# anshumang/gunrockINST

Hardware: AMD Instinct MI355X
Metric: MTEPS (million traversed edges/sec) BFS R-MAT scale-24 (higher is better)
Workload: dtype int32; 1 GPU; BFS idempotent direction-optimizing (traversal_mode 2), R-MAT scale-24 (a=.55 b=.2 c=.2 d=.05, 8 pairs/vertex mirrored, seed 0x6772): n=16777216, m=265395436 directed edges; sources: largest-degree + 64 seeded; search_depth_src0=7, max_degree=218420

## Files before the change

### gunrockinst_amd/csrc/gunrock/app/bfs/bfs_enactor.hpp

```cpp
#pragma once

#include <hip/hip_runtime.h>
#include <cstdlib>

#include <gunrock/app/bfs/bfs_functor.hpp>
#include <gunrock/app/bfs/bfs_problem.hpp>
#include <gunrock/app/enactor_base.hpp>
#include <gunrock/oprtr/advance/bottom_up.hpp>
#include <gunrock/oprtr/advance/kernel.hpp>
#include <gunrock/oprtr/advance/twc.hpp>
#include <gunrock/util/context.hpp>

namespace gunrock {
namespace app {
namespace bfs {

template <bool INSTRUMENT>
class BFSEnactor : public EnactorBase {
   public:
    explicit BFSEnactor(bool DEBUG = false) : EnactorBase(VERTEX_FRONTIERS, DEBUG) {}
    ~BFSEnactor() override {}

    void GetKernelStatistics(long long &launches, double &kernel_ms)
    {
// ... 188 lines not shown
                    if (scap > cu_count * 4) scap = cu_count * 4;
                    if (sgrid > scap) sgrid = scap;
                    hipLaunchKernelGGL((oprtr::advance::BottomUpSparseKernel<BU_THREADS, 8, 32, BFSProblem, L, true>),
                                       dim3(static_cast<unsigned>(sgrid)), dim3(BU_THREADS), 0, stream, bargs, *ds, lookup);
                    queue_emitted = true;
                    return util::GRError("BottomUpSparseKernel launch failed", __FILE__, __LINE__);
                }
                const long long scap = max_grid_size > 0 ? max_grid_size
                    : util::ResidentGrid(oprtr::advance::BottomUpSparseKernel<BU_THREADS, 8, 32, BFSProblem, L, false>, BU_THREADS);
                if (sgrid > scap) sgrid = scap;
                hipLaunchKernelGGL((oprtr::advance::BottomUpSparseKernel<BU_THREADS, 8, 32, BFSProblem, L, false>),
                                   dim3(static_cast<unsigned>(sgrid)), dim3(BU_THREADS), 0, stream, bargs, *ds, lookup);
                return util::GRError("BottomUpSparseKernel launch failed", __FILE__, __LINE__);
            }
            if (heads_only) {
                typedef oprtr::advance::BitmapLookup<VertexId> L;
                const long long hcap = max_grid_size > 0 ? max_grid_size : util::ResidentGrid(oprtr::advance::BottomUpHeadsKernel<BU_THREADS, BFSProblem, L>, BU_THREADS);
                if (grid > hcap) grid = hcap;
                if (grid < 1) grid = 1;
                hipLaunchKernelGGL((oprtr::advance::BottomUpHeadsKernel<BU_THREADS, BFSProblem, L>), dim3(static_cast<unsigned>(grid)), dim3(BU_THREADS), 0,
                                   stream, bargs, *ds, lookup);
                return util::GRError("BottomUpHeadsKernel launch failed", __FILE__, __LINE__);
            }
            const long long cap = max_grid_size > 0 ? max_grid_size
                : util::ResidentGrid(oprtr::advance::BottomUpKernel<BU_THREADS, 8, 32, BFSProblem, oprtr::advance::BitmapLookup<VertexId>>, BU_THREADS);
            if (grid > cap) grid = cap;
            if (grid < 1) grid = 1;
            hipLaunchKernelGGL((oprtr::advance::BottomUpKernel<BU_THREADS, 8, 32, BFSProblem, oprtr::advance::BitmapLookup<VertexId>>),
                               dim3(static_cast<unsigned>(grid)), dim3(BU_THREADS), 0, stream, bargs, *ds, lookup);
            return util::GRError("BottomUpKernel launch failed", __FILE__, __LINE__);
        };
        const int chain_len = (dobfs && problem->chain_sweeps > 0)
            ? (problem->chain_sweeps < oprtr::advance::kChainMax ? problem->chain_sweeps : oprtr::advance::kChainMax) : 0;
        work_progress.publish_sets = chain_len > 0 ? chain_len + 1 : 1;
        oprtr::advance::SweepRule sweep_rule;
        sweep_rule.with_in_edges = problem->with_in_edges;
        sweep_rule.nodes = problem->nodes;
        sweep_rule.beta = problem->beta;
        sweep_rule.emit_factor = problem->emit_queue_factor;
        sweep_rule.sparse_div = problem->sparse_sweep_div;
        auto run_sweep_chain = [&](long long first_in) -> hipError_t {
            typedef oprtr::advance::BitmapLookup<VertexId> L;
            hipError_t rc = hipSuccess;
            const long long it0 = iteration;
            const long long base_total = enactor_stats.total_queued;
            int masks[oprtr::advance::kChainMax + 1];
            masks[0] = cur_mask;
            int queued = 0;
            const long long bu_steps = ((static_cast<long long>(problem->nodes) + 63) / 64 + oprtr::advance::kBottomUpStepWords - 1) / oprtr::advance::kBottomUpStepWords;
            long long grid = (bu_steps + (BU_THREADS / 64) - 1) / (BU_THREADS / 64);
            const long long cap = max_grid_size > 0 ? max_grid_size
                : util::ResidentGrid(oprtr::advance::BottomUpAutoKernel<BU_THREADS, 8, 32, BFSProblem, L>, BU_THREADS);
            if (grid > cap) grid = cap;
            if (grid < 1) grid = 1;
            const long long chunks = ((static_cast<long long>(problem->nodes) + 63) / 64 + oprtr::advance::kSparseChunkWords - 1) / oprtr::advance::kSparseChunkWords;
            long long sparse_grid = (chunks + (BU_THREADS / 64) - 1) / (BU_THREADS / 64);
            if (sparse_grid < 1) sparse_grid = 1;
            long long emit_grid = sparse_grid < cu_count * 4 ? sparse_grid : cu_count * 4;
            for (int k = 1; k <= chain_len; ++k) {
                bool got = false;
                if ((rc = problem->TryAcquireMask(stream, masks[k], masks, k, got))) return rc;
                if (!got) break;
                oprtr::advance::BottomUpArgs<VertexId, SizeT> bargs;
                bargs.nodes = problem->nodes;
                bargs.d_inv_row_offsets = ds->d_inv_row_offsets;
                bargs.d_inv_column_indices = ds->d_inv_column_indices;
                bargs.d_inv_heads = ds->d_inv_heads;
                L lookup{ds->d_frontier_mask[masks[k - 1]]};
                bargs.d_frontier_out = reinterpret_cast<unsigned long long *>(ds->d_frontier_mask[masks[k]]);
                bargs.d_visited = reinterpret_cast<unsigned long long *>(ds->d_visited_mask);
                const long long level = it0 + k - 1;
                bargs.d_tail_out = work_progress.d_tail + ((level + 1) & 3);
                bargs.d_tail_clear = work_progress.d_tail + ((level + 2) & 3);
                bargs.d_wide = work_progress.d_wide + static_cast<size_t>(k) * util::WorkProgress::kWideSetWords;
                bargs.head_skip = 0;
                bargs.heads_only = 0;
                bargs.d_never = reinterpret_cast<const unsigned long long *>(ds->d_never_mask);
                bargs.d_head_base = ds->d_head_base;
                bargs.d_duty = INSTRUMENT ? DutySlot() : nullptr;
                bargs.queue_out = gs->frontier_queues[selector];
                bargs.d_fwd_row_offsets = gs->d_row_offsets;
                bargs.d_queue_tail = work_progress.d_tail + ((level + 1) & 3);
                bargs.d_queue_invalid = reinterpret_cast<int *>(work_progress.AuxTail());
                bargs.d_overflow = work_progress.d_overflow;
                oprtr::advance::SweepChain chain;
                chain.d_sets = work_progress.d_wide;
                chain.base_total = base_total;
                chain.first_in = first_in;
                chain.rule = sweep_rule;
                chain.index = k;
                chain.first_may_switch = 0;
                chain.d_log = work_progress.d_chain_log;
                typename BFSProblem::DataSlice level_slice = *ds;
                level_slice.iteration = static_cast<VertexId>(level);
                hipLaunchKernelGGL((oprtr::advance::BottomUpAutoKernel<BU_THREADS, 8, 32, BFSProblem, L>), dim3(static_cast<unsigned>(grid)),
                                   dim3(BU_THREADS), 0, stream, bargs, level_slice, lookup, chain, static_cast<unsigned>(sparse_grid),
                                   static_cast<unsigned>(emit_grid));
                if ((rc = util::GRError("BottomUpAutoKernel launch failed", __FILE__, __LINE__))) return rc;
                queued = k;
            }
            if (queued == 0) return util::GRError(hipErrorInvalidValue, "BFSEnactor: no frontier bitmap for a bottom-up sweep", __FILE__, __LINE__);
            const bool closing_queued = problem->chain_closing && problem->persistent_edge_limit > 0;
            int *d_gate = work_progress.d_chain_log + 8;
            bool emit_queued = false;
            if (closing_queued) {
                oprtr::advance::PersistentArgs<VertexId, SizeT> p;
                p.t.queue[0] = gs->frontier_queues[0];
                p.t.queue[1] = gs->frontier_queues[1];
                p.t.selector = selector;
                p.t.first_iteration = it0;
                p.t.d_tail = work_progress.d_tail;
                p.t.max_levels = kTailMaxLevels;
                p.t.d_levels_done = work_progress.LevelsDone();
                p.t.d_level_sums = work_progress.d_sums;
                p.t.d_row_offsets = gs->d_row_offsets;
                p.t.d_column_indices = gs->d_column_indices;
                p.t.d_overflow = work_progress.d_overflow;
                p.t.edge_limit = static_cast<SizeT>(static_cast<long long>(problem->persistent_edge_limit) * 4);
                p.barrier.d_counter = work_progress.BarrierCounter();
                p.barrier.d_timeout = work_progress.BarrierTimeout();
// ... 368 lines not shown
```

### gunrockinst_amd/csrc/gunrock/app/bfs/bfs_problem.hpp

```cpp
#pragma once

#include <hip/hip_runtime.h>

#include <gunrock/app/problem_base.hpp>
#include <gunrock/graphio/device_csr.hpp>
#include <gunrock/graphio/relabel.hpp>
#include <gunrock/oprtr/advance/binned.hpp>
#include <gunrock/oprtr/advance/bottom_up.hpp>
#include <gunrock/util/memset_kernel.hpp>

namespace gunrock {
namespace app {
namespace bfs {

template <typename SizeT>
__global__ void NoInEdgeMaskKernel(const SizeT *d_inv_row_offsets, long long nodes, long long words64, unsigned long long *d_mask)
{
    const unsigned lane = threadIdx.x & 63;
    const long long wave0 = (static_cast<long long>(blockIdx.x) * blockDim.x + threadIdx.x) / 64;
    const long long nwaves = static_cast<long long>(gridDim.x) * blockDim.x / 64;
    for (long long w = wave0; w < words64; w += nwaves) {
        const long long v = w * 64 + lane;
        const bool none = v < nodes && d_inv_row_offsets[v + 1] == d_inv_row_offsets[v];
        const unsigned long long m = __ballot(none);
// ... 809 lines not shown
        }
        return src_row[1] - src_row[0];
    }

    hipError_t Extract(VertexId *h_labels, VertexId *h_preds)
    {
        hipError_t retval = hipSuccess;
        hipStream_t stream = this->graph_slices[0]->stream;
        GR_CHECK(FinishSearch(stream), "BFSProblem Extract: label pass failed");
        GR_CHECK(hipStreamSynchronize(stream), "BFSProblem Extract sync failed");
        if (this->nodes > 0)
            GR_CHECK(hipMemcpy(h_labels, d_out_labels, sizeof(VertexId) * static_cast<size_t>(this->nodes), hipMemcpyDeviceToHost),
                     "BFSProblem hipMemcpy d_labels failed");
        if (MARK_PREDECESSORS && h_preds && this->nodes > 0)
            GR_CHECK(hipMemcpy(h_preds, d_out_preds, sizeof(VertexId) * static_cast<size_t>(this->nodes), hipMemcpyDeviceToHost),
                     "BFSProblem hipMemcpy d_preds failed");
        return retval;
    }

    bool defer_labels = true;
    bool emit_current = false;
    bool labels_deferred = false;
    int label_pass = 1;
    int level_mask_limit = kLevelMasks;
    LevelMaskList<VertexId> level_masks;
    int mask_ring = 0;

    bool MaskKept(int idx) const
    {
        for (int k = 0; k < level_masks.count; ++k)
            if (level_masks.mask[k] == reinterpret_cast<const unsigned long long *>(data_slices[0]->d_frontier_mask[idx])) return true;
        return false;
    }
    hipError_t AcquireMask(hipStream_t stream, int &idx, int hold_a = -1, int hold_b = -1)
    {
        const int holds[2] = {hold_a, hold_b};
        bool got = false;
        const hipError_t rc = TryAcquireMask(stream, idx, holds, 2, got);
        if (rc) return rc;
        return got ? hipSuccess : util::GRError(hipErrorInvalidValue, "BFSProblem: no free frontier bitmap", __FILE__, __LINE__);
    }
    hipError_t TryAcquireMask(hipStream_t stream, int &idx, const int *holds, int n_holds, bool &got)
    {
        hipError_t retval = hipSuccess;
        got = true;
        if (!data_slices[0]->d_frontier_mask[1]) {
// ... 155 lines not shown
```

### gunrockinst_amd/csrc/gunrock/oprtr/advance/bottom_up.hpp

```cpp
#pragma once

#include <hip/hip_runtime.h>

#include <gunrock/oprtr/advance/sweep_chain.hpp>
#include <gunrock/oprtr/frontier_writer.hpp>
#include <gunrock/util/device_intrinsics.hpp>
#include <gunrock/util/error_utils.hpp>
#include <gunrock/util/frontier.hpp>
#include <gunrock/util/kernel_runtime_stats.hpp>

namespace gunrock {
namespace oprtr {
namespace advance {

template <typename VertexId, typename SizeT>
__global__ void QueueToBitmapKernel(const VertexId *d_queue, SizeT length, unsigned *d_bitmap)
{
    const SizeT stride = static_cast<SizeT>(gridDim.x) * blockDim.x;
    for (SizeT i = static_cast<SizeT>(blockIdx.x) * blockDim.x + threadIdx.x; i < length; i += stride) {
        const VertexId v = d_queue[i];
        atomicOr(d_bitmap + (static_cast<unsigned>(v) >> 5), 1u << (v & 31));
    }
}

// ... 115 lines not shown
    unsigned long long *d_queue_tail = nullptr;
    int *d_queue_invalid = nullptr;
    int *d_overflow = nullptr;
    int heads_only = 0;
    unsigned long long *d_wide = nullptr;
    unsigned long long *d_duty = nullptr;
};

#ifndef GRX_BU_STEP_WORDS
#define GRX_BU_STEP_WORDS 8
#endif
constexpr int kBottomUpStepWords = GRX_BU_STEP_WORDS;
#ifndef GRX_BU_SPARSE_CHUNK_WORDS
#define GRX_BU_SPARSE_CHUNK_WORDS 64
#endif
constexpr int kSparseChunkWords = GRX_BU_SPARSE_CHUNK_WORDS;

struct __attribute__((packed, aligned(4))) Quad {
    int v[4];
};

constexpr int kHeadScan = 512;

template <typename VertexId, typename SizeT>
__global__ void BuildHeadsKernel(const SizeT *d_row_offsets, const VertexId *d_column_indices, long long nodes, int2 *d_heads,
                                 const SizeT *d_degree_offsets,
                                 const unsigned long long *d_never = nullptr, const unsigned *d_head_base = nullptr)
{
    const unsigned lane = util::LaneId();
    const long long nwaves = static_cast<long long>(gridDim.x) * blockDim.x / util::kWaveSize;
    for (long long v = (static_cast<long long>(blockIdx.x) * blockDim.x + threadIdx.x) / util::kWaveSize; v < nodes; v += nwaves) {
        const SizeT b = d_row_offsets[v], e = d_row_offsets[v + 1];
        const SizeT len = (e - b < kHeadScan) ? e - b : kHeadScan;
        unsigned long long k1 = 0, k2 = 0;
        for (SizeT i = lane; i < len; i += util::kWaveSize) {
            const VertexId u = d_column_indices[b + i];
            const unsigned long long deg = d_degree_offsets ? static_cast<unsigned long long>(d_degree_offsets[u + 1] - d_degree_offsets[u])
                                                            : static_cast<unsigned long long>(kHeadScan - i);
            const unsigned long long k = ((deg + 1) << 32) | static_cast<unsigned>(u);
            if (k > k1) { k2 = k1; k1 = k; }
            else if (k > k2) k2 = k;
        }
        unsigned long long best1 = k1;
        for (int o = 32; o; o >>= 1) {
            const unsigned long long other = __shfl_xor(best1, o, util::kWaveSize);
            best1 = other > best1 ? other : best1;
        }
        unsigned long long best2 = (k1 == best1) ? k2 : k1;
        for (int o = 32; o; o >>= 1) {
            const unsigned long long other = __shfl_xor(best2, o, util::kWaveSize);
            best2 = other > best2 ? other : best2;
        }
        if (lane == 0) {
            int2 h;
            h.x = best1 ? static_cast<int>(static_cast<unsigned>(best1)) : -1;
            h.y = best2 ? static_cast<int>(static_cast<unsigned>(best2)) : -1;
            if (!d_head_base) {
                d_heads[v] = h;
            } else if (e > b) {
                const unsigned long long with_edges = ~d_never[v >> 6];
                d_heads[d_head_base[v >> 6] + __popcll(with_edges & ((1ull << (v & 63)) - 1ull))] = h;
            }
        }
    }
}

template <int PROBE, int SOLO_LIMIT, typename VertexId, typename SizeT, typename Lookup>
__device__ __forceinline__ VertexId WalkRow(const BottomUpArgs<VertexId, SizeT> &a, const Lookup &in_frontier, bool active, VertexId v,
                                            unsigned lane, VertexId known_a = -1, VertexId known_b = -1, bool extent_given = false,
                                            SizeT given_begin = 0, SizeT given_end = 0)
{
    SizeT pos = 0, end = 0;
    VertexId p_found = -1;
    if (extent_given) {
        pos = given_begin + a.head_skip;
        end = given_end;
    } else if (active) {
        pos = a.d_inv_row_offsets[v] + a.head_skip;
        end = a.d_inv_row_offsets[v + 1];
// ... 113 lines not shown
                    head[j] = a.d_inv_heads[open ? idx : 0u];
                }
            } else {
#pragma unroll
                for (int j = 0; j < STEP_WORDS; ++j) {
                    const unsigned long long open_mask = __shfl(my_open, j, util::kWaveSize);
                    const bool open = (open_mask >> lane) & 1ull;
                    open_bits |= static_cast<unsigned>(open) << j;
                    const long long v = (step * STEP_WORDS + j) * 64 + lane;
                    head[j] = a.d_inv_heads[open ? v : 0];
                }
            }
            bool hit[STEP_WORDS];
#pragma unroll
            for (int j = 0; j < STEP_WORDS; ++j) {
                const bool ask = ((open_bits >> j) & 1u) && head[j].x >= 0;
                hit[j] = in_frontier(ask ? head[j].x : 0) && ask;
            }
            VertexId parent[STEP_WORDS];
            unsigned ask_y = 0;
#pragma unroll
            for (int j = 0; j < STEP_WORDS; ++j) {
                parent[j] = hit[j] ? head[j].x : static_cast<VertexId>(-1);
                if (((open_bits >> j) & 1u) && head[j].x >= 0 && !hit[j] && head[j].y >= 0) ask_y |= 1u << j;
            }
            unsigned more_bits = 0;
            if (__ballot(ask_y != 0) != 0) {
#pragma unroll
                for (int j = 0; j < STEP_WORDS; ++j) {
                    const bool ask = (ask_y >> j) & 1u;
                    hit[j] = in_frontier(ask ? head[j].y : 0) && ask;
                }
#pragma unroll
                for (int j = 0; j < STEP_WORDS; ++j) {
                    if (hit[j]) parent[j] = head[j].y;
                    if (((ask_y >> j) & 1u) && !hit[j]) more_bits |= 1u << j;
                }
            }

            if (HEADS_ONLY || a.heads_only) more_bits = 0;
            typedef typename ProblemData::SizeT SizeT;
            SizeT next_begin = 0, next_end = 0;
            if (!HEADS_ONLY && more_bits != 0) {
                const long long nv = (step * STEP_WORDS + (__ffs(more_bits) - 1)) * 64 + lane;
                next_begin = a.d_inv_row_offsets[nv];
                next_end = a.d_inv_row_offsets[nv + 1];
            }
            while (!HEADS_ONLY && __ballot(more_bits != 0) != 0) {
                const bool active = more_bits != 0;
                const int jl = active ? (__ffs(more_bits) - 1) : 0;
                more_bits &= more_bits - 1;
                const VertexId v = static_cast<VertexId>((step * STEP_WORDS + jl) * 64 + lane);
                const SizeT row_begin = next_begin, row_end = next_end;
                if (more_bits != 0) {
                    const long long nv = (step * STEP_WORDS + (__ffs(more_bits) - 1)) * 64 + lane;
                    next_begin = a.d_inv_row_offsets[nv];
                    next_end = a.d_inv_row_offsets[nv + 1];
                }
                VertexId hx = -1, hy = -1;
// ... 30 lines not shown
                const unsigned long long fm = __ballot(found);
                if (static_cast<int>(lane) == j) my_found |= fm;
            }
        }
        if (owns_word) {
            a.d_frontier_out[my_word] = my_found;
            if (my_found) a.d_visited[my_word] = my_vis | my_found;
        }
    }

    unsigned long long packed = util::PackTail(found_count, found_edges);
    packed = util::WaveSum(packed);
    if (lane == 0) s_total[tid / util::kWaveSize] = packed;
    __syncthreads();
    if (tid == 0) {
        unsigned long long sum = 0;
#pragma unroll
        for (int i = 0; i < WAVES; ++i) sum += s_total[i];
        unsigned long long *slot = util::WideTailSlot(a.d_wide);
        if (sum) atomicAdd(slot ? slot : a.d_tail_out, sum);
    }
}

#ifndef GRX_BU_MIN_WAVES
#define GRX_BU_MIN_WAVES 6
#endif
template <int THREADS, int PROBE, int SOLO_LIMIT, typename ProblemData, typename Lookup>
__global__ __launch_bounds__(THREADS, GRX_BU_MIN_WAVES) void BottomUpKernel(
    BottomUpArgs<typename ProblemData::VertexId, typename ProblemData::SizeT> a, typename ProblemData::DataSlice slice,
    Lookup in_frontier)
{
    DenseSweep<THREADS, PROBE, SOLO_LIMIT, ProblemData, Lookup>(a, slice, in_frontier);
}

#ifndef GRX_BU_HEADS_MIN_WAVES
#define GRX_BU_HEADS_MIN_WAVES 6
#endif
template <int THREADS, typename ProblemData, typename Lookup>
__global__ __launch_bounds__(THREADS, GRX_BU_HEADS_MIN_WAVES) void BottomUpHeadsKernel(
    BottomUpArgs<typename ProblemData::VertexId, typename ProblemData::SizeT> a, typename ProblemData::DataSlice slice,
    Lookup in_frontier)
{
    DenseSweep<THREADS, 8, 32, ProblemData, Lookup, true>(a, slice, in_frontier);
}

__device__ __forceinline__ int NthSetBit(unsigned long long x, int r)
{
    int pos = 0;
#pragma unroll
    for (int s = 32; s; s >>= 1) {
        const int c = __popcll(x & (((1ull << s) - 1ull) << pos));
        if (r >= c) {
            r -= c;
            pos += s;
        }
// ... 57 lines not shown
            my_with_edges = ~a.d_never[my_word];
            my_base = a.d_head_base[my_word];
        }
        for (int i = lane; i < CHUNK_WORDS * 2; i += util::kWaveSize) s_found[wave][i] = 0;
        __builtin_amdgcn_wave_barrier();

        for (unsigned base = 0; base < total; base += util::kWaveSize) {
            const unsigned k = base + lane;
            const bool active = k < total;
            int j = 0;
#pragma unroll
            for (int s = CHUNK_WORDS / 2; s; s >>= 1)
                if (__shfl(inc, j + s - 1, util::kWaveSize) <= k) j += s;
            if (!active) j = 0;
            const unsigned before = __shfl(inc, j, util::kWaveSize) - __shfl(cnt, j, util::kWaveSize);
            const unsigned long long open_j = __shfl(my_open, j, util::kWaveSize);
            const int bit = active ? NthSetBit(open_j, static_cast<int>(k - before)) : 0;
            const VertexId v = static_cast<VertexId>((chunk * CHUNK_WORDS + j) * 64 + bit);
            long long head_index = v;
            if (a.d_head_base) {
                const unsigned long long we = __shfl(my_with_edges, j, util::kWaveSize);
                head_index = __shfl(my_base, j, util::kWaveSize) + __popcll(we & ((1ull << bit) - 1ull));
            }
            const int2 head = a.d_inv_heads[active ? head_index : 0];
            VertexId parent = -1;
            const bool ask_x = active && head.x >= 0;
            const bool hit_x = in_frontier(ask_x ? head.x : 0) && ask_x;
            if (hit_x) parent = head.x;
            const bool ask_y = ask_x && !hit_x && head.y >= 0;
            bool more = false;
            if (__ballot(ask_y) != 0) {
                const bool hit_y = in_frontier(ask_y ? head.y : 0) && ask_y;
                if (hit_y) parent = head.y;
                more = ask_y && !hit_y;
            }
            if (a.heads_only) more = false;
            if (__ballot(more) != 0) {
                const VertexId late = WalkRow<PROBE, SOLO_LIMIT>(a, in_frontier, more, v, lane, head.x, head.y);
                if (more && late >= 0) parent = late;
            }
            if (parent >= 0) {
                if (!slice.defer_labels) slice.d_labels[v] = new_label;
                if (ProblemData::MARK_PREDECESSORS) slice.d_preds[v] = parent;
                atomicOr(&s_found[wave][2 * j + (bit >> 5)], 1u << (bit & 31));
            }
            if (EMIT_QUEUE && emit) {
                const unsigned long long fm = __ballot(parent >= 0);
                if (fm) {
                    const int leader = __ffsll(static_cast<long long>(fm)) - 1;
                    int at = 0;
                    if (static_cast<int>(lane) == leader) at = atomicAdd(&s_writer.count, __popcll(fm));
                    at = __shfl(at, leader, util::kWaveSize);
                    if (parent >= 0 && at + __popcll(fm) <= CAPACITY) s_writer.buf[at + util::RankInMask(fm)] = v;
                }
            }
        }
        __builtin_amdgcn_wave_barrier();
// ... 16 lines not shown
        for (int i = 0; i < WAVES; ++i) sum += s_total[i];
        unsigned long long *slot = util::WideTailSlot(a.d_wide);
        if (sum) atomicAdd(slot ? slot : a.d_tail_out, sum);
    }
    if (EMIT_QUEUE && emit) {
        const int staged = Writer::Count(s_writer);
        __syncthreads();
        if (staged > CAPACITY) {
            if (tid == 0) *a.d_queue_invalid = 1;
        } else {
            Writer::template Flush<true>(s_writer, staged, a.queue_out, a.d_queue_tail, a.d_overflow, a.d_fwd_row_offsets);
        }
    }
}

template <int THREADS, int PROBE, int SOLO_LIMIT, typename ProblemData, typename Lookup, bool EMIT_QUEUE>
__global__ __launch_bounds__(THREADS) void BottomUpSparseKernel(
    BottomUpArgs<typename ProblemData::VertexId, typename ProblemData::SizeT> a, typename ProblemData::DataSlice slice,
    Lookup in_frontier)
{
    SparseSweep<THREADS, PROBE, SOLO_LIMIT, ProblemData, Lookup, EMIT_QUEUE>(a, slice, in_frontier, EMIT_QUEUE, gridDim.x);
}

template <int THREADS, int PROBE, int SOLO_LIMIT, typename ProblemData, typename Lookup>
__global__ __launch_bounds__(THREADS, GRX_BU_MIN_WAVES) void BottomUpAutoKernel(
    BottomUpArgs<typename ProblemData::VertexId, typename ProblemData::SizeT> a, typename ProblemData::DataSlice slice,
    Lookup in_frontier, SweepChain chain, unsigned sparse_grid, unsigned emit_grid)
{
    const int action = ChainAction(chain, util::LaneId());
    if (blockIdx.x == 0 && threadIdx.x == 0) {
        chain.d_log[chain.index] = action;
        if (action >= kSweepDense && action != kSweepSparseEmit && a.d_queue_tail) *a.d_queue_tail = 0ull;
    }
    if (action < kSweepDense) return;
    if (action == kSweepDense) {
        DenseSweep<THREADS, PROBE, SOLO_LIMIT, ProblemData, Lookup>(a, slice, in_frontier);
    } else {
        const unsigned want = action == kSweepSparseEmit ? emit_grid : sparse_grid;
        const unsigned limit = want < gridDim.x ? want : gridDim.x;
        if (blockIdx.x >= limit) return;
        SparseSweep<THREADS, PROBE, SOLO_LIMIT, ProblemData, Lookup, true>(a, slice, in_frontier, action == kSweepSparseEmit, limit);
    }
}

template <int THREADS, typename VertexId, typename SizeT>
__global__ __launch_bounds__(THREADS) void BitmapToQueueKernel(const unsigned *d_bitmap, SizeT nodes,
                                                               util::Frontier<VertexId, SizeT> out,
                                                               unsigned long long *d_tail_out, int *d_overflow,
                                                               const SizeT *d_row_offsets)
{
    constexpr int CAPACITY = 16 * THREADS;
    constexpr int WAVES = THREADS / util::kWaveSize;
    typedef FrontierWriter<THREADS, CAPACITY, VertexId, SizeT> Writer;
    __shared__ typename Writer::Storage s_writer;
    __shared__ unsigned s_pop[WAVES];

    const long long words = (static_cast<long long>(nodes) + 31) / 32;
    const long long per_wg = ((words + gridDim.x - 1) / gridDim.x + THREADS - 1) / THREADS * THREADS;
    const long long w_begin = static_cast<long long>(blockIdx.x) * per_wg;
// ... 66 lines not shown
```

### gunrockinst_amd/csrc/lib/bfs_app.hip

```cpp
#include <gunrock/gunrock.h>
#include <gunrock/gunrock_mi355x.h>

#include <cstdio>
#include <cstdlib>

#include <gunrock/app/bfs/bfs_enactor.hpp>
#include <gunrock/app/bfs/bfs_problem.hpp>
#include <gunrock/app/handle_runner.hpp>
#include <gunrock/graphio/device_sort.hpp>
#include <gunrock/graphio/symmetry.hpp>
#include <gunrock/oprtr/filter/kernel.hpp>
#include <gunrock/csr.hpp>
#include <gunrock/graphio/utils.hpp>
#include <gunrock/util/context.hpp>

using namespace gunrock;
using namespace gunrock::app;
using namespace gunrock::app::bfs;

namespace {

struct BfsRunner {
    virtual ~BfsRunner() {}
    virtual hipError_t Init(const Csr<int, int, int> &g) = 0;
// ... 76 lines not shown
    }
    void FreeInverse()
    {
        if (d_inv_row_offsets) util::GRError(hipFree(d_inv_row_offsets), "BFS hipFree inverse offsets failed", __FILE__, __LINE__);
        if (d_inv_column_indices) util::GRError(hipFree(d_inv_column_indices), "BFS hipFree inverse columns failed", __FILE__, __LINE__);
        d_inv_row_offsets = nullptr;
        d_inv_column_indices = nullptr;
    }
    int *d_inv_row_offsets = nullptr;
    int *d_inv_column_indices = nullptr;
    void SetPersistentLimit(int limit) override { problem.persistent_edge_limit = limit; }
    void SetTwcLimit(int limit) override { problem.twc_edge_limit = limit; }
    void SetCooperativeLaunch(bool on) override { problem.cooperative_launch = on; }
    void SetBinnedMinEdges(long long min_edges) override { problem.binned_min_edges = min_edges; }
    int SetOption(const char *name, double value) override
    {
        const std::string key(name ? name : "");
        if (key == "emit_queue_factor") problem.emit_queue_factor = static_cast<float>(value);
        else if (key == "sparse_sweep_div") problem.sparse_sweep_div = static_cast<int>(value);
        else if (key == "speculative_emit") problem.speculative_emit = value != 0.0;
        else if (key == "chain_sweeps") problem.chain_sweeps = static_cast<int>(value);
        else if (key == "chain_closing") problem.chain_closing = value != 0.0;
        else if (key == "label_pass") problem.label_pass = value != 0.0 ? 1 : 0;
        else if (key == "relabel") {
            if (value > 0.0 && !problem.HasRelabelled()) return 2;
            problem.relabel = value > 0.0 ? 1 : (value < 0.0 ? -1 : 0);
        } else if (key == "relabel_min_nodes") {
            if (value < 0.0) return 2;
            problem.relabel_min_nodes = static_cast<long long>(value);
        } else if (key == "relabel_hubs") {
            if (value < 0.0) return 2;
            const long long hubs = static_cast<long long>(value);
            if (!problem.HasRelabelled()) problem.relabel_hubs = hubs;
            else if (hubs != problem.relabel_hubs && problem.BuildRelabelled(hubs) != hipSuccess) return 3;
        } else return 1;
        return 0;
    }
    void BuildRelabelled(bool on) override { problem.build_relabelled = on; }
    long long MaskFlushes() override { return problem.mask_flushes; }
    void RelabelInfo(long long &hubs, long long &with_edges, int &threshold, float &build_ms, long long &bytes) override
    {
        const bool ready = problem.HasRelabelled();
        hubs = ready ? problem.relabelled.hubs : -1;
        with_edges = ready ? problem.relabelled.with_edges : -1;
        threshold = ready ? problem.relabelled.threshold : 0;
        build_ms = ready ? problem.relabelled.build_ms : 0.f;
// ... 358 lines not shown
```

### gunrockinst_amd/csrc/lib/partitioned_bfs.hip

```cpp
#include <gunrock/gunrock_mi355x.h>

#include <dlfcn.h>
#include <cstdio>
#include <cstring>
#include <string>
#include <vector>

#include <gunrock/app/bfs/bfs_problem.hpp>
#include <gunrock/app/enactor_base.hpp>
#include <gunrock/app/problem_base.hpp>
#include <gunrock/graphio/device_sort.hpp>
#include <gunrock/oprtr/advance/bottom_up.hpp>
#include <gunrock/oprtr/advance/kernel.hpp>
#include <gunrock/oprtr/filter/kernel.hpp>
#include <gunrock/util/memset_kernel.hpp>

using namespace gunrock;

namespace {

struct ncclUniqueIdBytes {
    char internal[128];
};

// ... 390 lines not shown
    {
        if (hipStreamSynchronize(stream) != hipSuccess) return -1;
        return gather(ctx, d_send, d_recv, words);
    }
    int AllToAllV(const int *d_send, const size_t *sc, const size_t *so, int *d_recv, const size_t *rc, const size_t *ro,
                  hipStream_t stream) override
    {
        if (hipStreamSynchronize(stream) != hipSuccess) return -1;
        return a2a(ctx, d_send, sc, so, d_recv, rc, ro);
    }
    const char *Name() const override { return "callbacks"; }
};

struct Pbfs : app::EnactorBase {
    int parts = 1, rank = 0;
    int n_global = 0, n_local = 0, n_local_max = 0, m_local = 0;
    int *d_row_offsets = nullptr, *d_col_indices = nullptr;
    PbfsProblem::DataSlice ds{};
    unsigned *d_frontier_mask[2] = {nullptr, nullptr};
    int2 *d_heads = nullptr;
    unsigned *d_never = nullptr;
    unsigned *d_head_base = nullptr;
    long long with_in_edges = 0;
    int sparse_sweep_div = 6;
    bool never_applied = false;
    util::Frontier<int, int> queues[2];
    int *d_candidates = nullptr, *d_send = nullptr;
    unsigned *d_counts = nullptr, *h_counts = nullptr;
    int candidate_capacity = 0;
    hipStream_t stream = 0;
    int selector = 0, cur_mask = 0;
    unsigned frontier_len = 0, frontier_edges = 0;
    int level = 0;
    Transport *transport = nullptr;
    bool mark_pred = false;
    double alpha = 12.0;
    long long m_global = -1;
    int *d_recv = nullptr;
    int recv_capacity = 0;
    int *d_send_preds = nullptr;
    unsigned *d_small = nullptr;
    unsigned *h_small = nullptr;
    unsigned long long mail_seq = 0;
    unsigned *d_mark_bits = nullptr;
    double lite_factor = 230.0;
    long long marked_levels = 0;
// ... 279 lines not shown
        b.head_skip = 0;
        b.d_never = reinterpret_cast<const unsigned long long *>(d_never);
        b.d_head_base = d_head_base;
        b.d_frontier_out = reinterpret_cast<unsigned long long *>(d_frontier_mask[cur_mask ^ 1]);
        b.d_visited = reinterpret_cast<unsigned long long *>(ds.d_visited_mask);
        b.d_tail_out = work_progress.d_tail + 1;
        b.d_tail_clear = nullptr;
        b.d_wide = work_progress.d_wide;
        ds.iteration = level;
        L lookup{d_gathered_masks, static_cast<unsigned>(parts), static_cast<unsigned>(words_per_rank)};
        const long long words64 = (static_cast<long long>(n_local) + 63) / 64;
        if (sparse_sweep_div > 0 && open_estimate >= 0 && open_estimate * sparse_sweep_div <= static_cast<long long>(n_local)) {
            long long sgrid = ((words64 + oprtr::advance::kSparseChunkWords - 1) / oprtr::advance::kSparseChunkWords + 3) / 4;
            const long long scap = util::ResidentGrid(oprtr::advance::BottomUpSparseKernel<256, 8, 32, PbfsProblem, L, false>, 256);
            if (sgrid > scap) sgrid = scap;
            if (sgrid < 1) sgrid = 1;
            hipLaunchKernelGGL((oprtr::advance::BottomUpSparseKernel<256, 8, 32, PbfsProblem, L, false>), dim3(static_cast<unsigned>(sgrid)),
                               dim3(256), 0, stream, b, ds, lookup);
            GR_CHECK(hipGetLastError(), "BottomUpSparseKernel launch failed");
            return retval;
        }
        const long long bu_steps = (words64 + oprtr::advance::kBottomUpStepWords - 1) / oprtr::advance::kBottomUpStepWords;
        long long grid = (bu_steps + 3) / 4;
        const long long cap = util::ResidentGrid(oprtr::advance::BottomUpKernel<256, 8, 32, PbfsProblem, L>, 256);
        if (grid > cap) grid = cap;
        if (grid < 1) grid = 1;
        hipLaunchKernelGGL((oprtr::advance::BottomUpKernel<256, 8, 32, PbfsProblem, L>), dim3(static_cast<unsigned>(grid)), dim3(256), 0, stream,
                           b, ds, lookup);
        GR_CHECK(hipGetLastError(), "BottomUpKernel launch failed");
        return retval;
    }

    hipError_t BitmapToQueue(unsigned *len, unsigned *edges)
    {
        hipError_t retval = hipSuccess;
        if ((retval = work_progress.ClearAux(stream))) return retval;
        hipLaunchKernelGGL((oprtr::advance::BitmapToQueueKernel<256, int, int>), dim3(cu_count * 4), dim3(256), 0, stream,
                           d_frontier_mask[cur_mask], n_local, queues[selector], work_progress.AuxTail(), work_progress.d_overflow,
                           d_row_offsets);
        GR_CHECK(hipGetLastError(), "BitmapToQueueKernel launch failed");
        if ((retval = work_progress.GetAux(frontier_len, frontier_edges, stream))) return retval;
        *len = frontier_len;
        *edges = frontier_edges;
        return retval;
    }

    hipError_t PrepareSearch()
    {
        hipError_t retval = hipSuccess;
        if (!transport) return hipErrorNotInitialized;
        if (!d_small) {
// ... 328 lines not shown
}

int grx_pbfs_labels(grx_pbfs *p, int **d_labels)
{
    if (!p || !d_labels) return -1;
    *d_labels = p->impl.ds.d_labels;
    return 0;
}

int grx_pbfs_preds(grx_pbfs *p, int **d_preds)
{
    if (!p || !d_preds) return -1;
    *d_preds = p->impl.ds.d_preds;
    return 0;
}

int grx_pbfs_set_option(grx_pbfs *p, const char *name, double value)
{
    if (!p || !name) return -1;
    const std::string key(name);
    if (key == "lite_factor") p->impl.lite_factor = value;
    else if (key == "alpha") p->impl.alpha = value;
    else if (key == "sparse_sweep_div") p->impl.sparse_sweep_div = static_cast<int>(value);
    else return 1;
    return 0;
}

long long grx_pbfs_stat(grx_pbfs *p, const char *name)
{
    if (!p || !name) return -1;
    const std::string key(name);
    if (key == "marked_levels") return p->impl.marked_levels;
    return -1;
}

int grx_rccl_load(void)
{
    return RcclApi::Get().Load() ? 0 : -2;
}

int grx_rccl_unique_id(char id[128])
{
    if (!id) return -1;
    RcclApi &api = RcclApi::Get();
    if (!api.Load()) return -2;
    ncclUniqueIdBytes uid;
// ... 52 lines not shown
```

Baseline: 966,300 MTEPS.

## Queue bottom-up row walkers in LDS and drain them wave-wide across batches

Adds a queued dense bottom-up sweep. Vertices whose two cached heads both miss are pushed into a per-wave shared-memory ring and walked together once enough accumulate, instead of walking each step's few unresolved vertices at low lane occupancy. It also encodes in the heads table when the second head is the vertex's last in-edge, so those vertices skip the row walk entirely. The queued path is on by default and adds shared-memory footprint and wave barriers, which may lower occupancy.

```diff
diff --git a/gunrockinst_amd/csrc/gunrock/app/bfs/bfs_enactor.hpp b/gunrockinst_amd/csrc/gunrock/app/bfs/bfs_enactor.hpp
--- a/gunrockinst_amd/csrc/gunrock/app/bfs/bfs_enactor.hpp
+++ b/gunrockinst_amd/csrc/gunrock/app/bfs/bfs_enactor.hpp
@@ -234,12 +234,19 @@
                                    stream, bargs, *ds, lookup);
                 return util::GRError("BottomUpHeadsKernel launch failed", __FILE__, __LINE__);
             }
+            typedef oprtr::advance::BitmapLookup<VertexId> L;
+            const bool walk_queue = problem->walk_queue != 0;
             const long long cap = max_grid_size > 0 ? max_grid_size
-                : util::ResidentGrid(oprtr::advance::BottomUpKernel<BU_THREADS, 8, 32, BFSProblem, oprtr::advance::BitmapLookup<VertexId>>, BU_THREADS);
+                : walk_queue ? util::ResidentGrid(oprtr::advance::BottomUpKernel<BU_THREADS, 8, 32, BFSProblem, L, true>, BU_THREADS)
+                             : util::ResidentGrid(oprtr::advance::BottomUpKernel<BU_THREADS, 8, 32, BFSProblem, L, false>, BU_THREADS);
             if (grid > cap) grid = cap;
             if (grid < 1) grid = 1;
-            hipLaunchKernelGGL((oprtr::advance::BottomUpKernel<BU_THREADS, 8, 32, BFSProblem, oprtr::advance::BitmapLookup<VertexId>>),
-                               dim3(static_cast<unsigned>(grid)), dim3(BU_THREADS), 0, stream, bargs, *ds, lookup);
+            if (walk_queue)
+                hipLaunchKernelGGL((oprtr::advance::BottomUpKernel<BU_THREADS, 8, 32, BFSProblem, L, true>),
+                                   dim3(static_cast<unsigned>(grid)), dim3(BU_THREADS), 0, stream, bargs, *ds, lookup);
+            else
+                hipLaunchKernelGGL((oprtr::advance::BottomUpKernel<BU_THREADS, 8, 32, BFSProblem, L, false>),
+                                   dim3(static_cast<unsigned>(grid)), dim3(BU_THREADS), 0, stream, bargs, *ds, lookup);
             return util::GRError("BottomUpKernel launch failed", __FILE__, __LINE__);
         };
         const int chain_len = (dobfs && problem->chain_sweeps > 0)
@@ -261,8 +268,10 @@
             int queued = 0;
             const long long bu_steps = ((static_cast<long long>(problem->nodes) + 63) / 64 + oprtr::advance::kBottomUpStepWords - 1) / oprtr::advance::kBottomUpStepWords;
             long long grid = (bu_steps + (BU_THREADS / 64) - 1) / (BU_THREADS / 64);
+            const bool walk_queue = problem->walk_queue != 0;
             const long long cap = max_grid_size > 0 ? max_grid_size
-                : util::ResidentGrid(oprtr::advance::BottomUpAutoKernel<BU_THREADS, 8, 32, BFSProblem, L>, BU_THREADS);
+                : walk_queue ? util::ResidentGrid(oprtr::advance::BottomUpAutoKernel<BU_THREADS, 8, 32, BFSProblem, L, true>, BU_THREADS)
+                             : util::ResidentGrid(oprtr::advance::BottomUpAutoKernel<BU_THREADS, 8, 32, BFSProblem, L, false>, BU_THREADS);
             if (grid > cap) grid = cap;
             if (grid < 1) grid = 1;
             const long long chunks = ((static_cast<long long>(problem->nodes) + 63) / 64 + oprtr::advance::kSparseChunkWords - 1) / oprtr::advance::kSparseChunkWords;
@@ -305,9 +314,14 @@
                 chain.d_log = work_progress.d_chain_log;
                 typename BFSProblem::DataSlice level_slice = *ds;
                 level_slice.iteration = static_cast<VertexId>(level);
-                hipLaunchKernelGGL((oprtr::advance::BottomUpAutoKernel<BU_THREADS, 8, 32, BFSProblem, L>), dim3(static_cast<unsigned>(grid)),
-                                   dim3(BU_THREADS), 0, stream, bargs, level_slice, lookup, chain, static_cast<unsigned>(sparse_grid),
-                                   static_cast<unsigned>(emit_grid));
+                if (walk_queue)
+                    hipLaunchKernelGGL((oprtr::advance::BottomUpAutoKernel<BU_THREADS, 8, 32, BFSProblem, L, true>), dim3(static_cast<unsigned>(grid)),
+                                       dim3(BU_THREADS), 0, stream, bargs, level_slice, lookup, chain, static_cast<unsigned>(sparse_grid),
+                                       static_cast<unsigned>(emit_grid));
+                else
+                    hipLaunchKernelGGL((oprtr::advance::BottomUpAutoKernel<BU_THREADS, 8, 32, BFSProblem, L, false>), dim3(static_cast<unsigned>(grid)),
+                                       dim3(BU_THREADS), 0, stream, bargs, level_slice, lookup, chain, static_cast<unsigned>(sparse_grid),
+                                       static_cast<unsigned>(emit_grid));
                 if ((rc = util::GRError("BottomUpAutoKernel launch failed", __FILE__, __LINE__))) return rc;
                 queued = k;
             }
diff --git a/gunrockinst_amd/csrc/gunrock/app/bfs/bfs_problem.hpp b/gunrockinst_amd/csrc/gunrock/app/bfs/bfs_problem.hpp
--- a/gunrockinst_amd/csrc/gunrock/app/bfs/bfs_problem.hpp
+++ b/gunrockinst_amd/csrc/gunrock/app/bfs/bfs_problem.hpp
@@ -855,6 +855,7 @@
     bool emit_current = false;
     bool labels_deferred = false;
     int label_pass = 1;
+    int walk_queue = 1;
     int level_mask_limit = kLevelMasks;
     LevelMaskList<VertexId> level_masks;
     int mask_ring = 0;
diff --git a/gunrockinst_amd/csrc/gunrock/oprtr/advance/bottom_up.hpp b/gunrockinst_amd/csrc/gunrock/oprtr/advance/bottom_up.hpp
--- a/gunrockinst_amd/csrc/gunrock/oprtr/advance/bottom_up.hpp
+++ b/gunrockinst_amd/csrc/gunrock/oprtr/advance/bottom_up.hpp
@@ -161,6 +161,10 @@
 
 constexpr int kHeadScan = 512;
 
+__host__ __device__ __forceinline__ int EncodeLastHead(int id) { return -2 - id; }
+__device__ __forceinline__ int HeadId(int stored) { return stored < -1 ? -2 - stored : stored; }
+__device__ __forceinline__ bool HeadIsLast(int stored) { return stored < -1; }
+
 template <typename VertexId, typename SizeT>
 __global__ void BuildHeadsKernel(const SizeT *d_row_offsets, const VertexId *d_column_indices, long long nodes, int2 *d_heads,
                                  const SizeT *d_degree_offsets,
@@ -194,6 +198,7 @@
             int2 h;
             h.x = best1 ? static_cast<int>(static_cast<unsigned>(best1)) : -1;
             h.y = best2 ? static_cast<int>(static_cast<unsigned>(best2)) : -1;
+            if (e - b == 2 && h.y >= 0) h.y = EncodeLastHead(h.y);
             if (!d_head_base) {
                 d_heads[v] = h;
             } else if (e > b) {
@@ -353,19 +358,19 @@
 #pragma unroll
             for (int j = 0; j < STEP_WORDS; ++j) {
                 parent[j] = hit[j] ? head[j].x : static_cast<VertexId>(-1);
-                if (((open_bits >> j) & 1u) && head[j].x >= 0 && !hit[j] && head[j].y >= 0) ask_y |= 1u << j;
+                if (((open_bits >> j) & 1u) && head[j].x >= 0 && !hit[j] && head[j].y != -1) ask_y |= 1u << j;
             }
             unsigned more_bits = 0;
             if (__ballot(ask_y != 0) != 0) {
 #pragma unroll
                 for (int j = 0; j < STEP_WORDS; ++j) {
                     const bool ask = (ask_y >> j) & 1u;
-                    hit[j] = in_frontier(ask ? head[j].y : 0) && ask;
+                    hit[j] = in_frontier(ask ? HeadId(head[j].y) : 0) && ask;
                 }
 #pragma unroll
                 for (int j = 0; j < STEP_WORDS; ++j) {
-                    if (hit[j]) parent[j] = head[j].y;
-                    if (((ask_y >> j) & 1u) && !hit[j]) more_bits |= 1u << j;
+                    if (hit[j]) parent[j] = HeadId(head[j].y);
+                    if (((ask_y >> j) & 1u) && !hit[j] && !HeadIsLast(head[j].y)) more_bits |= 1u << j;
                 }
             }
 
@@ -442,15 +447,217 @@
     }
 }
 
+#ifndef GRX_BU_WALK_BATCH
+#define GRX_BU_WALK_BATCH 4
+#endif
+#ifndef GRX_BU_WALK_DRAIN
+#define GRX_BU_WALK_DRAIN 64
+#endif
+constexpr int kWalkBatch = GRX_BU_WALK_BATCH;
+constexpr int kWalkDrain = GRX_BU_WALK_DRAIN;
+constexpr int kWalkQueue = 128;
+
+template <int THREADS, int PROBE, int SOLO_LIMIT, typename ProblemData, typename Lookup>
+__device__ __forceinline__ void DenseSweepQueued(const BottomUpArgs<typename ProblemData::VertexId, typename ProblemData::SizeT> &a,
+                                                 typename ProblemData::DataSlice &slice, const Lookup &in_frontier)
+{
+    typedef typename ProblemData::VertexId VertexId;
+    typedef typename ProblemData::SizeT SizeT;
+    constexpr int WAVES = THREADS / util::kWaveSize;
+    constexpr int STEP_WORDS = kBottomUpStepWords;
+    constexpr int BATCH_WORDS = kWalkBatch * STEP_WORDS;
+    static_assert(BATCH_WORDS <= util::kWaveSize && (STEP_WORDS & (STEP_WORDS - 1)) == 0, "one bitmap word of the batch per lane; a step's lanes are an aligned group");
+    static_assert(kWalkDrain >= 1 && kWalkDrain <= util::kWaveSize, "a round is at most one entry per lane");
+    static_assert((kWalkDrain - 1) + util::kWaveSize <= kWalkQueue, "the queue holds what waits plus one word's append");
+    static_assert((kWalkQueue & (kWalkQueue - 1)) == 0, "ring positions are masked");
+    static_assert(BATCH_WORDS * 64 <= 65536, "an entry names its vertex by (word of the batch, bit)");
+    __shared__ unsigned long long s_total[WAVES];
+    __shared__ unsigned s_found[WAVES][BATCH_WORDS * 2];
+    __shared__ unsigned long long s_visited[WAVES][BATCH_WORDS];
+    __shared__ unsigned long long s_open[WAVES][BATCH_WORDS];
+    __shared__ unsigned long long s_with_edges[WAVES][BATCH_WORDS];
+    __shared__ unsigned s_base[WAVES][BATCH_WORDS];
+    __shared__ unsigned short s_walker[WAVES][kWalkQueue];
+    util::DutyStamp duty(a.d_duty);
+
+    const int tid = threadIdx.x;
+    const unsigned lane = util::LaneId();
+    const unsigned wave = tid / util::kWaveSize;
+    if (blockIdx.x == 0 && tid == 0 && a.d_tail_clear) *a.d_tail_clear = 0ull;
+
+    const long long words = (static_cast<long long>(a.nodes) + 63) / 64;
+    const long long steps = (words + STEP_WORDS - 1) / STEP_WORDS;
+    const long long wave0 = (static_cast<long long>(blockIdx.x) * THREADS + tid) / util::kWaveSize;
+    const long long nwaves = static_cast<long long>(gridDim.x) * WAVES;
+    const VertexId new_label = slice.iteration + 1;
+
+    unsigned found_count = 0;
+    unsigned q_read = 0, q_count = 0;
+    for (long long first = wave0; first < steps; first += nwaves * kWalkBatch) {
+        auto drain = [&](unsigned take) {
+            const bool active = lane < take;
+            const unsigned at = (q_read + lane) & (kWalkQueue - 1);
+            const unsigned code = s_walker[wave][at];
+            const unsigned w = code >> 6, bit = code & 63u;
+            const VertexId v = static_cast<VertexId>(((first + (w / STEP_WORDS) * nwaves) * STEP_WORDS + (w % STEP_WORDS)) * 64 + bit);
+            SizeT row_begin = 0, row_end = 0;
+            if (active) {
+                row_begin = a.d_inv_row_offsets[v];
+                row_end = a.d_inv_row_offsets[v + 1];
+            }
+            const VertexId p_found = WalkRow<PROBE, SOLO_LIMIT>(a, in_frontier, active, v, lane, -1, -1, true, row_begin, row_end);
+            if (active && p_found >= 0) {
+                if (!slice.defer_labels) slice.d_labels[v] = new_label;
+                if (ProblemData::MARK_PREDECESSORS) slice.d_preds[v] = p_found;
+                atomicOr(&s_found[wave][2 * w + (bit >> 5)], 1u << (bit & 31u));
+            }
+            q_read += take;
+            q_count -= take;
+            __builtin_amdgcn_wave_barrier();
+        };
+
+        const long long my_step = first + static_cast<long long>(lane / STEP_WORDS) * nwaves;
+        const long long my_word = my_step * STEP_WORDS + (lane % STEP_WORDS);
+        const bool owns_word = lane < BATCH_WORDS && my_step < steps && my_word < words;
+        unsigned long long my_open = 0ull;
+        if (owns_word) my_open = ~a.d_visited[my_word];
+        if (lane < BATCH_WORDS) s_visited[wave][lane] = ~my_open;
+        if (owns_word && (my_word + 1) * 64 > a.nodes) {
+            const int valid = static_cast<int>(a.nodes - my_word * 64);
+            my_open &= (valid >= 64) ? ~0ull : ((1ull << valid) - 1ull);
+        }
+        const unsigned long long open_words = __ballot(my_open != 0);
+        if (lane < BATCH_WORDS) {
+            s_open[wave][lane] = my_open;
+            if (a.d_head_base) {
+                s_with_edges[wave][lane] = owns_word ? ~a.d_never[my_word] : 0ull;
+                s_base[wave][lane] = owns_word ? a.d_head_base[my_word] : 0u;
+            }
+        }
+        __builtin_amdgcn_wave_barrier();
+
+#pragma unroll 1
+        for (int b = 0; b < kWalkBatch; ++b) {
+            if (((open_words >> (b * STEP_WORDS)) & ((1ull << STEP_WORDS) - 1ull)) == 0) continue;
+            const long long step = first + b * nwaves;
+            int2 head[STEP_WORDS];
+            unsigned open_bits = 0;
+            if (a.d_head_base) {
+#pragma unroll
+                for (int j = 0; j < STEP_WORDS; ++j) {
+                    const unsigned long long open_mask = s_open[wave][b * STEP_WORDS + j];
+                    const bool open = (open_mask >> lane) & 1ull;
+                    open_bits |= static_cast<unsigned>(open) << j;
+                    const unsigned long long we = s_with_edges[wave][b * STEP_WORDS + j];
+                    const unsigned idx = s_base[wave][b * STEP_WORDS + j] + static_cast<unsigned>(__popcll(we & ((1ull << lane) - 1ull)));
+                    head[j] = a.d_inv_heads[open ? idx : 0u];
+                }
+            } else {
+#pragma unroll
+                for (int j = 0; j < STEP_WORDS; ++j) {
+                    const unsigned long long open_mask = s_open[wave][b * STEP_WORDS + j];
+                    const bool open = (open_mask >> lane) & 1ull;
+                    open_bits |= static_cast<unsigned>(open) << j;
+                    const long long v = (step * STEP_WORDS + j) * 64 + lane;
+                    head[j] = a.d_inv_heads[open ? v : 0];
+                }
+            }
+            bool hit[STEP_WORDS];
+#pragma unroll
+            for (int j = 0; j < STEP_WORDS; ++j) {
+                const bool ask = ((open_bits >> j) & 1u) && head[j].x >= 0;
+                hit[j] = in_frontier(ask ? head[j].x : 0) && ask;
+            }
+            VertexId parent[STEP_WORDS];
+            unsigned ask_y = 0;
+#pragma unroll
+            for (int j = 0; j < STEP_WORDS; ++j) {
+                parent[j] = hit[j] ? head[j].x : static_cast<VertexId>(-1);
+                if (((open_bits >> j) & 1u) && head[j].x >= 0 && !hit[j] && head[j].y != -1) ask_y |= 1u << j;
+            }
+            unsigned more_bits = 0;
+            if (__ballot(ask_y != 0) != 0) {
+#pragma unroll
+                for (int j = 0; j < STEP_WORDS; ++j) {
+                    const bool ask = (ask_y >> j) & 1u;
+                    hit[j] = in_frontier(ask ? HeadId(head[j].y) : 0) && ask;
+                }
+#pragma unroll
+                for (int j = 0; j < STEP_WORDS; ++j) {
+                    if (hit[j]) parent[j] = HeadId(head[j].y);
+                    if (((ask_y >> j) & 1u) && !hit[j] && !HeadIsLast(head[j].y)) more_bits |= 1u << j;
+                }
+            }
+            if (a.heads_only) more_bits = 0;
+
+            unsigned long long head_found = 0;
+#pragma unroll
+            for (int j = 0; j < STEP_WORDS; ++j) {
+                const bool found = parent[j] >= 0;
+                if (found) {
+                    const VertexId v = static_cast<VertexId>((step * STEP_WORDS + j) * 64 + lane);
+                    if (!slice.defer_labels) slice.d_labels[v] = new_label;
+                    if (ProblemData::MARK_PREDECESSORS) slice.d_preds[v] = parent[j];
+                }
+                const unsigned long long fm = __ballot(found);
+                if (static_cast<int>(lane) == j) head_found = fm;
+            }
+            if (lane < STEP_WORDS) {
+                s_found[wave][2 * (b * STEP_WORDS + lane)] = static_cast<unsigned>(head_found);
+                s_found[wave][2 * (b * STEP_WORDS + lane) + 1] = static_cast<unsigned>(head_found >> 32);
+            }
+            __builtin_amdgcn_wave_barrier();
+
+#pragma unroll 1
+            for (int j = 0; j < STEP_WORDS; ++j) {
+                const bool walker = (more_bits >> j) & 1u;
+                const unsigned long long wm = __ballot(walker);
+                if (wm == 0) continue;
+                if (walker) {
+                    const unsigned at = (q_read + q_count + util::RankInMask(wm)) & (kWalkQueue - 1);
+                    s_walker[wave][at] = static_cast<unsigned short>(((b * STEP_WORDS + j) << 6) | lane);
+                }
+                q_count += static_cast<unsigned>(__popcll(wm));
+                __builtin_amdgcn_wave_barrier();
+                while (q_count >= kWalkDrain) drain(q_count < util::kWaveSize ? q_count : util::kWaveSize);
+            }
+        }
+        while (q_count != 0) drain(q_count < util::kWaveSize ? q_count : util::kWaveSize);
+        if (owns_word) {
+            const bool step_ran = ((open_words >> (lane & ~static_cast<unsigned>(STEP_WORDS - 1))) & ((1ull << STEP_WORDS) - 1ull)) != 0;
+            unsigned long long f = 0ull;
+            if (step_ran)
+                f = static_cast<unsigned long long>(s_found[wave][2 * lane]) | (static_cast<unsigned long long>(s_found[wave][2 * lane + 1]) << 32);
+            a.d_frontier_out[my_word] = f;
+            if (f) a.d_visited[my_word] = s_visited[wave][lane] | f;
+            found_count += static_cast<unsigned>(__popcll(f));
+        }
+        __builtin_amdgcn_wave_barrier();
+    }
+
+    unsigned long long packed = util::PackTail(found_count, 0u);
+    packed = util::WaveSum(packed);
+    if (lane == 0) s_total[tid / util::kWaveSize] = packed;
+    __syncthreads();
+    if (tid == 0) {
+        unsigned long long sum = 0;
+#pragma unroll
+        for (int i = 0; i < WAVES; ++i) sum += s_total[i];
+        unsigned long long *slot = util::WideTailSlot(a.d_wide);
+        if (sum) atomicAdd(slot ? slot : a.d_tail_out, sum);
+    }
+}
+
 #ifndef GRX_BU_MIN_WAVES
 #define GRX_BU_MIN_WAVES 6
 #endif
-template <int THREADS, int PROBE, int SOLO_LIMIT, typename ProblemData, typename Lookup>
+template <int THREADS, int PROBE, int SOLO_LIMIT, typename ProblemData, typename Lookup, bool WALK_QUEUE = true>
 __global__ __launch_bounds__(THREADS, GRX_BU_MIN_WAVES) void BottomUpKernel(
     BottomUpArgs<typename ProblemData::VertexId, typename ProblemData::SizeT> a, typename ProblemData::DataSlice slice,
     Lookup in_frontier)
 {
-    DenseSweep<THREADS, PROBE, SOLO_LIMIT, ProblemData, Lookup>(a, slice, in_frontier);
+    if (WALK_QUEUE) DenseSweepQueued<THREADS, PROBE, SOLO_LIMIT, ProblemData, Lookup>(a, slice, in_frontier);
+    else DenseSweep<THREADS, PROBE, SOLO_LIMIT, ProblemData, Lookup>(a, slice, in_frontier);
 }
 
 #ifndef GRX_BU_HEADS_MIN_WAVES
@@ -554,7 +761,9 @@
                 const unsigned long long we = __shfl(my_with_edges, j, util::kWaveSize);
                 head_index = __shfl(my_base, j, util::kWaveSize) + __popcll(we & ((1ull << bit) - 1ull));
             }
-            const int2 head = a.d_inv_heads[active ? head_index : 0];
+            int2 head = a.d_inv_heads[active ? head_index : 0];
+            const bool last_head = HeadIsLast(head.y);
+            head.y = HeadId(head.y);
             VertexId parent = -1;
             const bool ask_x = active && head.x >= 0;
             const bool hit_x = in_frontier(ask_x ? head.x : 0) && ask_x;
@@ -564,7 +773,7 @@
             if (__ballot(ask_y) != 0) {
                 const bool hit_y = in_frontier(ask_y ? head.y : 0) && ask_y;
                 if (hit_y) parent = head.y;
-                more = ask_y && !hit_y;
+                more = ask_y && !hit_y && !last_head;
             }
             if (a.heads_only) more = false;
             if (__ballot(more) != 0) {
@@ -627,7 +836,7 @@
     SparseSweep<THREADS, PROBE, SOLO_LIMIT, ProblemData, Lookup, EMIT_QUEUE>(a, slice, in_frontier, EMIT_QUEUE, gridDim.x);
 }
 
-template <int THREADS, int PROBE, int SOLO_LIMIT, typename ProblemData, typename Lookup>
+template <int THREADS, int PROBE, int SOLO_LIMIT, typename ProblemData, typename Lookup, bool WALK_QUEUE = true>
 __global__ __launch_bounds__(THREADS, GRX_BU_MIN_WAVES) void BottomUpAutoKernel(
     BottomUpArgs<typename ProblemData::VertexId, typename ProblemData::SizeT> a, typename ProblemData::DataSlice slice,
     Lookup in_frontier, SweepChain chain, unsigned sparse_grid, unsigned emit_grid)
@@ -639,7 +848,8 @@
     }
     if (action < kSweepDense) return;
     if (action == kSweepDense) {
-        DenseSweep<THREADS, PROBE, SOLO_LIMIT, ProblemData, Lookup>(a, slice, in_frontier);
+        if (WALK_QUEUE) DenseSweepQueued<THREADS, PROBE, SOLO_LIMIT, ProblemData, Lookup>(a, slice, in_frontier);
+        else DenseSweep<THREADS, PROBE, SOLO_LIMIT, ProblemData, Lookup>(a, slice, in_frontier);
     } else {
         const unsigned want = action == kSweepSparseEmit ? emit_grid : sparse_grid;
         const unsigned limit = want < gridDim.x ? want : gridDim.x;
diff --git a/gunrockinst_amd/csrc/lib/bfs_app.hip b/gunrockinst_amd/csrc/lib/bfs_app.hip
--- a/gunrockinst_amd/csrc/lib/bfs_app.hip
+++ b/gunrockinst_amd/csrc/lib/bfs_app.hip
@@ -122,6 +122,7 @@
         else if (key == "chain_sweeps") problem.chain_sweeps = static_cast<int>(value);
         else if (key == "chain_closing") problem.chain_closing = value != 0.0;
         else if (key == "label_pass") problem.label_pass = value != 0.0 ? 1 : 0;
+        else if (key == "walk_queue") problem.walk_queue = value != 0.0 ? 1 : 0;
         else if (key == "relabel") {
             if (value > 0.0 && !problem.HasRelabelled()) return 2;
             problem.relabel = value > 0.0 ? 1 : (value < 0.0 ? -1 : 0);
diff --git a/gunrockinst_amd/csrc/lib/partitioned_bfs.hip b/gunrockinst_amd/csrc/lib/partitioned_bfs.hip
--- a/gunrockinst_amd/csrc/lib/partitioned_bfs.hip
+++ b/gunrockinst_amd/csrc/lib/partitioned_bfs.hip
@@ -436,6 +436,7 @@
     unsigned *d_never = nullptr;
     unsigned *d_head_base = nullptr;
     long long with_in_edges = 0;
+    int walk_queue = 1;
     int sparse_sweep_div = 6;
     bool never_applied = false;
     util::Frontier<int, int> queues[2];
@@ -761,11 +762,16 @@
         }
         const long long bu_steps = (words64 + oprtr::advance::kBottomUpStepWords - 1) / oprtr::advance::kBottomUpStepWords;
         long long grid = (bu_steps + 3) / 4;
-        const long long cap = util::ResidentGrid(oprtr::advance::BottomUpKernel<256, 8, 32, PbfsProblem, L>, 256);
+        const long long cap = walk_queue ? util::ResidentGrid(oprtr::advance::BottomUpKernel<256, 8, 32, PbfsProblem, L, true>, 256)
+                                         : util::ResidentGrid(oprtr::advance::BottomUpKernel<256, 8, 32, PbfsProblem, L, false>, 256);
         if (grid > cap) grid = cap;
         if (grid < 1) grid = 1;
-        hipLaunchKernelGGL((oprtr::advance::BottomUpKernel<256, 8, 32, PbfsProblem, L>), dim3(static_cast<unsigned>(grid)), dim3(256), 0, stream,
-                           b, ds, lookup);
+        if (walk_queue)
+            hipLaunchKernelGGL((oprtr::advance::BottomUpKernel<256, 8, 32, PbfsProblem, L, true>), dim3(static_cast<unsigned>(grid)), dim3(256), 0,
+                               stream, b, ds, lookup);
+        else
+            hipLaunchKernelGGL((oprtr::advance::BottomUpKernel<256, 8, 32, PbfsProblem, L, false>), dim3(static_cast<unsigned>(grid)), dim3(256), 0,
+                               stream, b, ds, lookup);
         GR_CHECK(hipGetLastError(), "BottomUpKernel launch failed");
         return retval;
     }
@@ -1140,6 +1146,7 @@
     if (key == "lite_factor") p->impl.lite_factor = value;
     else if (key == "alpha") p->impl.alpha = value;
     else if (key == "sparse_sweep_div") p->impl.sparse_sweep_div = static_cast<int>(value);
+    else if (key == "walk_queue") p->impl.walk_queue = value != 0.0 ? 1 : 0;
     else return 1;
     return 0;
 }
```

After: 1.013 million MTEPS (median of 6 runs). 4.9% higher.
